# matwilso/generative_models

Hardware: AMD Instinct MI355X
Metric: ddpm_train_images_per_sec (higher is better)
Workload: dtype fp16_fwd+bf16_bwd; 1 GPU; DDPM train step, 3x32x32, SimpleUnet C=128, 2048 images per GPU, T=1000 (BASELINE.json configs[2]); key=cfg2, global_batch=2048, parallelism=dp1

## Files before the change

generative_models_amd/csrc/conv1x1_stream.hip:

```cpp
#include <type_traits>

#include "gmk_common.h"
#include "conv_plan.h"

namespace {

constexpr int kRow = 272;

template <typename T>
__global__ __launch_bounds__(256) void conv1x1_pair_stream_kernel(const T* __restrict__ src, const T* __restrict__ w, T* __restrict__ out_a,
                                                                 T* __restrict__ out_b, unsigned npix, unsigned ntiles, unsigned src_bytes) {
    fp16_saturating_stores<T>();
    typedef typename Frag16<T>::type frag_t;
    typedef __attribute__((ext_vector_type(4))) unsigned int u32x4s;
    constexpr unsigned kBadOff = 0xFFFFFF00u;
    __shared__ __attribute__((aligned(16))) char wl[256 * kRow];
    __shared__ __attribute__((aligned(16))) char tile[128 * kRow];
    __shared__ __attribute__((aligned(16))) char trans[4 * 32 * kRow];
    const int tid = threadIdx.x, lane = tid & 63, wave = tid >> 6;
    const int r = lane & 31, h = lane >> 5;
    const __amdgpu_buffer_rsrc_t rss = __builtin_amdgcn_make_buffer_rsrc(const_cast<T*>(src), 0, (int)src_bytes, 0x00020000);
    const __amdgpu_buffer_rsrc_t rsa = __builtin_amdgcn_make_buffer_rsrc(out_a, 0, (int)src_bytes, 0x00020000);
    const __amdgpu_buffer_rsrc_t rsb = __builtin_amdgcn_make_buffer_rsrc(out_b, 0, (int)src_bytes, 0x00020000);
#pragma unroll
// ... 126 lines not shown
    if (nk > 0) {
        load_step(0, ry[0], rx0[0], rx1[0]);
        if (nk > 1) load_step(1, ry[1], rx0[1], rx1[1]);
        write_step(0, ry[0], rx0[0], rx1[0]);
    }
    __syncthreads();
    auto k_step = [&](int ks, auto par) {
        constexpr int PAR = decltype(par)::value;
        if (ks + 2 < nk) load_step(ks + 2, ry[PAR], rx0[PAR], rx1[PAR]);
        const char* Yb = smem + PAR * 49152;
        const char* Xb = Yb + 16384 + cib * 16384;
#pragma unroll
        for (int kk = 0; kk < 4; ++kk) {
            bf16x8 a[2], b[2];
            const int pxl = kk * 16 + 8 * hh + q;
#pragma unroll
            for (int i = 0; i < 2; ++i) {
                const int wa = (((wm * 2 + i) ^ q) << 6) + 32 * cblk + 8 * pp;
                const int wb = (((wn * 2 + i) ^ q) << 6) + 32 * cblk + 8 * pp;
                s16x4 lo = __builtin_amdgcn_ds_read_tr16_b64_v4i16((GMK_LDS s16x4*)(Yb + pxl * 256 + wa));
                s16x4 hi = __builtin_amdgcn_ds_read_tr16_b64_v4i16((GMK_LDS s16x4*)(Yb + (pxl + 4) * 256 + wa));
                const s16x8 t = {lo[0], lo[1], lo[2], lo[3], hi[0], hi[1], hi[2], hi[3]};
                a[i] = __builtin_bit_cast(bf16x8, t);
                lo = __builtin_amdgcn_ds_read_tr16_b64_v4i16((GMK_LDS s16x4*)(Xb + pxl * 256 + wb));
                hi = __builtin_amdgcn_ds_read_tr16_b64_v4i16((GMK_LDS s16x4*)(Xb + (pxl + 4) * 256 + wb));
                const s16x8 u = {lo[0], lo[1], lo[2], lo[3], hi[0], hi[1], hi[2], hi[3]};
                b[i] = __builtin_bit_cast(bf16x8, u);
            }
#pragma unroll
            for (int i = 0; i < 2; ++i)
#pragma unroll
                for (int j = 0; j < 2; ++j) acc[i][j] = __builtin_amdgcn_mfma_f32_32x32x16_bf16(a[i], b[j], acc[i][j], 0, 0, 0);
        }
        if (ks + 1 < nk) write_step(PAR ^ 1, ry[PAR ^ 1], rx0[PAR ^ 1], rx1[PAR ^ 1]);
        __syncthreads();
    };
    for (int ks = 0; ks < nk; ks += 2) {
        k_step(ks, std::integral_constant<int, 0>{});
        if (ks + 1 < nk) k_step(ks + 1, std::integral_constant<int, 1>{});
    }
    float* out = slab + (int64_t)blockIdx.x * (128 * 256) + cib * 128;
#pragma unroll
    for (int i = 0; i < 2; ++i)
#pragma unroll
        for (int j = 0; j < 2; ++j)
#pragma unroll
            for (int e = 0; e < 16; ++e) {
                const int co = wm * 64 + i * 32 + (e & 3) + 8 * (e >> 2) + 4 * h;
                const int ci = wn * 64 + j * 32 + r;
                out[co * 256 + ci] = acc[i][j][e];
            }
}

}

int gmk_conv1x1_pair_stream_try(const void* src, int64_t npix, const void* w_rows256, void* out_a, void* out_b, int dtype, void* stream) {
    if (!gmk_is16(dtype) || gmk_kernel_choice(3, "GMK_DEV_VARIANT") == 46) return 0;
    const int64_t bytes = npix * 256;
    if (bytes >= 0xFFFFFF00ll) return 0;
    const int64_t ntiles = (npix + 127) / 128;
    const int ncu = gmk_cu_limit();
    if (ntiles < 2 * ncu) return 0;
    const unsigned grid = (unsigned)ncu;
    if (dtype == GMK_BF16)
        conv1x1_pair_stream_kernel<bf16_t><<<grid, 256, 0, gmk_stream(stream)>>>((const bf16_t*)src, (const bf16_t*)w_rows256, (bf16_t*)out_a, (bf16_t*)out_b,
                                                                    (unsigned)npix, (unsigned)ntiles, (unsigned)bytes);
    else
        conv1x1_pair_stream_kernel<f16_t><<<grid, 256, 0, gmk_stream(stream)>>>((const f16_t*)src, (const f16_t*)w_rows256, (f16_t*)out_a, (f16_t*)out_b,
                                                                   (unsigned)npix, (unsigned)ntiles, (unsigned)bytes);
    return 1;
}

int gmk_conv1x1_wgrad_stream_try(const void* dy, int dy_cstride, const void* src0, const void* src1, int64_t npix, float* slab, int64_t slab_bytes,
                                 bool x_f16, void* stream) {
    if (gmk_kernel_choice(3, "GMK_DEV_VARIANT") == 47) return 0;
    const int ncu = gmk_cu_limit();
    if (npix < (int64_t)ncu * 64 * 8 || npix >= (1ll << 31) - 64) return 0;
    if (slab_bytes < (int64_t)ncu * 128 * 256 * 4) return 0;
    int64_t chunk = (npix + ncu - 1) / ncu;
    chunk = (chunk + 63) / 64 * 64;
    const int ns = (int)((npix + chunk - 1) / chunk);
    if (x_f16)
        conv1x1_wgrad_stream_kernel<f16_t><<<ns, 512, 0, gmk_stream(stream)>>>((const bf16_t*)dy, dy_cstride, (const f16_t*)src0, (const f16_t*)src1, slab, (int)npix, (int)chunk);
    else
        conv1x1_wgrad_stream_kernel<bf16_t><<<ns, 512, 0, gmk_stream(stream)>>>((const bf16_t*)dy, dy_cstride, (const bf16_t*)src0, (const bf16_t*)src1, slab, (int)npix, (int)chunk);
    return ns;
}
```

generative_models_amd/csrc/conv_igemm.hip:

```cpp
#include <stdlib.h>

#include <type_traits>

#include "gmk_common.h"
#include "conv_plan.h"

namespace {

constexpr int kBM = 128, kBN = 128;

struct GatherParams {
    int hs, ws;
    int ho, wo;
    int ksize, pad;
    int mul, shift, mask, lim_h, lim_w;
    signed char ty[9], tx[9];
    unsigned char tapw[9];
    int ntaps;
    int oscale, ooy, oox, out_w, out_hw;
};

__host__ bool make_gather(int mode, int ksize, int hs, int ws, int ho, int wo, GatherParams* g) {
    g->hs = hs; g->ws = ws; g->ho = ho; g->wo = wo;
    g->ksize = ksize; g->pad = ksize == 3 ? 1 : 0;
// ... 1093 lines not shown
    call.c0 = c0; call.c1 = c1; call.B = B; call.hs = call.ho = H; call.ws = call.wo = W; call.ksize = 3; call.mode = GMK_CONV_NORMAL;
    call.w_rows = call.cout = call.out_cstride = cout; call.dtype = GMK_BF16; call.gn_scale = call.gn_shift = true; call.gn_stride = c0 + c1;
    return gmk_conv_route(call, gmk_kernel_choice(0, "GMK_CONV_KERNEL"), gmk_subpixel_enabled()).route == GMK_ROUTE_HALO;
}

extern "C" int gmk_conv_wgrad(const void* dy, int dy_cstride, const void* src0, const void* src1, int c0, int c1, int B,
                              int hs, int ws, int ho, int wo, int ksize, int mode, float* dw, int cout, void* workspace,
                              int64_t workspace_bytes, int dtype, int x_dtype, void* stream) {
    GMK_REQUIRE(dy && src0 && dw && workspace, "gmk_conv_wgrad: null pointer");
    GMK_REQUIRE(dtype == GMK_BF16 || dtype == GMK_F32, "gmk_conv_wgrad: bad dtype %d", dtype);
    GMK_REQUIRE(x_dtype == dtype || (dtype == GMK_BF16 && x_dtype == GMK_F16),
                "gmk_conv_wgrad: activations of type %d with gradients of type %d (same type, or fp16 activations with bf16 gradients)", x_dtype, dtype);
    const bool xf16 = x_dtype == GMK_F16;
    GMK_REQUIRE(ksize == 1 || ksize == 3, "gmk_conv_wgrad: ksize %d", ksize);
    GMK_REQUIRE(c0 > 0 && c0 % 128 == 0 && c1 >= 0 && c1 % 128 == 0 && (c1 == 0 || src1),
                "gmk_conv_wgrad: source channels must be multiples of 128 (c0=%d c1=%d)", c0, c1);
    GMK_REQUIRE(cout > 0 && cout % 128 == 0 && dy_cstride >= cout, "gmk_conv_wgrad: bad cout=%d", cout);
    GMK_REQUIRE(B > 0 && (int64_t)B * ho * wo < (1ll << 31) - 256 && (int64_t)B * hs * ws < (1ll << 31),
                "gmk_conv_wgrad: problem too large for 32-bit pixel indices");
    GMK_REQUIRE(mode != GMK_CONV_TRANSPOSED2, "gmk_conv_wgrad: no weight gradient for the transposed gather");
    WgradParams p = {};
    GMK_REQUIRE(make_gather(mode, ksize, hs, ws, ho, wo, &p.g), "gmk_conv_wgrad: mode %d inconsistent with %dx%d -> %dx%d", mode, hs, ws, ho, wo);
    const int taps = ksize * ksize;
    const int wforce = gmk_kernel_choice(1, "GMK_WGRAD_KERNEL");
    const bool s2 = mode == GMK_CONV_STRIDE2 && hs == 2 * ho && ws == 2 * wo;
    if (wforce != 1 && dtype == GMK_BF16 && (mode == GMK_CONV_NORMAL || mode == GMK_CONV_UPSAMPLE2 || s2) && ksize == 3) {
        const int ns2 = gmk_conv_wgrad_slots_try(dy, dy_cstride, src0, src1, c0, c1, B, ho, wo, cout, (float*)workspace,
                                                 workspace_bytes, wforce, mode == GMK_CONV_UPSAMPLE2, xf16, stream, s2);
        if (ns2 > 0) return wgrad_reduce("gmk_conv_wgrad(slots)", (const float*)workspace, dw, ns2, taps, cout, c0 + c1, stream);
    }
    if (wforce != 1 && ksize == 1 && mode == GMK_CONV_NORMAL && dtype == GMK_BF16 && c0 == 128 && c1 == 128 && cout == 128) {
        const int ns1 = gmk_conv1x1_wgrad_stream_try(dy, dy_cstride, src0, src1, (int64_t)B * ho * wo, (float*)workspace, workspace_bytes, xf16, stream);
        if (ns1 > 0) {
            gmk_note_kernel(GMK_K_CONV1X1_WGRAD_STREAM);
            return wgrad_reduce("gmk_conv_wgrad(1x1 stream)", (const float*)workspace, dw, ns1, 1, cout, 256, stream);
        }
    }
    p.dy = dy; p.dy_cstride = dy_cstride; p.src0 = src0; p.src1 = src1; p.c0 = c0; p.c1 = c1; p.ktot = c0 + c1;
    p.cout = cout; p.M = B * ho * wo;
    const int ns = wgrad_nsplit(p.M, taps, cout, p.ktot, &p.chunk);
    const int64_t need = (int64_t)ns * taps * cout * p.ktot * 4;
    GMK_REQUIRE(workspace_bytes >= need, "gmk_conv_wgrad: workspace %lld < %lld bytes", (long long)workspace_bytes,
                (long long)need);
    p.slab = (float*)workspace;
    gmk_note_kernel(GMK_K_CONV_WGRAD);
    p.ns = ns; p.taps = taps; p.order = (gmk_kernel_choice(3, "GMK_DEV_VARIANT") & 0xFF) == 61;
    dim3 grid((ns + 7) / 8 * 8 * taps * (cout / 128) * (p.ktot / 128));
    if (dtype == GMK_BF16 && xf16) conv_wgrad_kernel<bf16_t, f16_t><<<grid, 256, 0, gmk_stream(stream)>>>(p);
    else if (dtype == GMK_BF16) conv_wgrad_kernel<bf16_t><<<grid, 256, 0, gmk_stream(stream)>>>(p);
    else if (fp32_split()) conv_wgrad_kernel<float, float, true><<<grid, 256, 0, gmk_stream(stream)>>>(p);
    else conv_wgrad_kernel<float><<<grid, 256, 0, gmk_stream(stream)>>>(p);
    return wgrad_reduce("gmk_conv_wgrad", p.slab, dw, ns, taps, cout, p.ktot, stream);
}
```

generative_models_amd/csrc/conv_plan.h:

```cpp
#pragma once
#include <stdint.h>

#include "../../include/gmk.h"

static inline bool gmk_fits32(int64_t bytes) { return bytes < 0xFFFF0000ll; }
static inline bool gmk_halo_family_allowed(int conv_choice) { return conv_choice == 0 || conv_choice == 3; }
static inline int gmk_xcd_splits(int ns) {
    if (ns >= 8) {
        const int all8 = ns & ~7, two = ns & ~3;
        ns = all8 * 16 < ns * 15 ? two : all8;
    }
    return ns < 1 ? 1 : ns;
}

struct HaloGeometry { int R, TP, slots; int64_t rows_total, M, ntiles, nb0, nb1, nbw, nbo; };
int gmk_halo_geometry(int B, int H, int W, int c0, int c1, int w_rows, int cout, int out_cstride, int min_tiles, int upsample,
                      int fused_gn, HaloGeometry* g);

void gmk_halo_schedule(int64_t ntiles, int cu_limit, int variant, bool fold, int* grid_x, int* nfull, int* nhalf);
int gmk_conv3x3_halo_try(const void* src0, const void* src1, int c0, int c1, int B, int H, int W, const void* w, int w_rows,
                         int n0, int cout, const float* bias, const float* emb, int emb_stride, const void* residual,
                         void* out, int out_cstride, int min_tiles, int upsample, float* stats, int64_t stats_bytes,
                         const float* gn_scale, const float* gn_shift, int gn_stride, int dtype, void* stream);

bool gmk_subpixel_enabled(void);
int gmk_subpixel_plan(int B, int H, int W, int cin, int cout, int w_rows, int ntaps, int out_cstride, HaloGeometry* g);
int gmk_subpixel_takes(int conv_choice, bool subpixel_on, int B, int H, int W, int cin, int cout, int w_rows, int ntaps, int out_cstride, int dtype);

enum ConvRoute {
    GMK_ROUTE_SUBPIXEL,
    GMK_ROUTE_HALO,
    GMK_ROUTE_PHASES,
    GMK_ROUTE_NEEDS_HALO,
    GMK_ROUTE_DMA,
    GMK_ROUTE_REG,
    GMK_ROUTE_TWO_CALLS
};
struct ConvCall {
    int c0, c1, B, hs, ws, ho, wo, ksize, mode, w_rows, n0, cout, out_cstride, dtype;
    bool emb, out2, gn_stats, gn_scale, gn_shift;
    int gn_stride;
};
struct ConvRoutePlan {
    ConvRoute route;
    bool stuffed;
    int halo_min_tiles, halo_upsample;
    int64_t nb0, nb1, nbw, nbo;
};
ConvRoutePlan gmk_conv_route(const ConvCall& c, int conv_choice, bool subpixel_on);

struct SlotPlan {
    int kernel;
    bool wide, share;
    bool auto_ok;
    int WE, RE, nchunks;
    int ns_cu, ns, cps;
    int grid[3];
    int64_t nbdy, nb0, nb1, slab_bytes;
};
int gmk_wgrad_slots_nsplit(int cout, int ktot, int cu_limit);
int gmk_wgrad_slot_plan(int B, int H, int W, int c0, int c1, int cout, int dy_cstride, int forced, int upsample, bool x_f16, int stride2,
                        int cu_limit, SlotPlan* plan);
int gmk_conv_wgrad_slots_try(const void* dy, int dy_cstride, const void* src0, const void* src1, int c0, int c1, int B, int H,
                             int W, int cout, float* slab, int64_t slab_bytes, int forced, int upsample, bool x_f16,
                             void* stream, int stride2 = 0);

struct SubWgradPlan { int ns, cps, nchunks; int grid[3]; int64_t slab_bytes; };
int gmk_wgrad_subpixel_plan(int B, int H, int W, int cin, int cout, int dy_cstride, int cu_limit, SubWgradPlan* plan);

int gmk_conv1x1_pair_stream_try(const void* src, int64_t npix, const void* w_rows256, void* out_a, void* out_b, int dtype, void* stream);
int gmk_conv1x1_wgrad_stream_try(const void* dy, int dy_cstride, const void* src0, const void* src1, int64_t npix, float* slab, int64_t slab_bytes,
                                 bool x_f16, void* stream);

struct SmallPlan {
    int kernel, launches;
    unsigned grid, block, lds;
    int ppb, tps, band, nbands, rows;
    unsigned nblocks, ntiles, ppw;
};
int gmk_expand_plan(int B, int cs, int H, int W, int C, int dtype, int variant, int cu_limit, SmallPlan* p);
int gmk_wgrad3_plan(int B, int cs, int H, int W, int C, int dtype, int variant, int cu_limit, SmallPlan* p);
int gmk_head_plan(int B, int cs, int H, int W, int C, int dtype, int variant, int cu_limit, bool stem_dgrad, SmallPlan* p);
```

generative_models_amd/diffusion/simple_unet.py:

```python
import math
import os
from collections import OrderedDict

import torch
from torch import nn

from .. import ops

MAX_TIMESTEPS = 256


def _res_names(prefix, cin, cout, emb):
    out = [
        (f"{prefix}.in_layers.0.weight", (cin,)), (f"{prefix}.in_layers.0.bias", (cin,)),
        (f"{prefix}.in_layers.2.weight", (cout, cin, 3, 3)), (f"{prefix}.in_layers.2.bias", (cout,)),
        (f"{prefix}.emb_layers.1.weight", (cout, emb)), (f"{prefix}.emb_layers.1.bias", (cout,)),
        (f"{prefix}.out_layers.0.weight", (cout,)), (f"{prefix}.out_layers.0.bias", (cout,)),
        (f"{prefix}.out_layers.3.weight", (cout, cout, 3, 3)), (f"{prefix}.out_layers.3.bias", (cout,)),
    ]
    if cin != cout:
        out += [(f"{prefix}.skip_connection.weight", (cout, cin, 1, 1)), (f"{prefix}.skip_connection.bias", (cout,))]
    return out


# ... 527 lines not shown

    def _wgrad(self, dy, srcs, ksize, mode, dw):
        self._on_side(lambda: ops.conv_wgrad(dy, srcs, ksize, mode, dw), (dy, *srcs))
        return dw

    def _on_side(self, fn, tensors):
        if not ops.WGRAD_STREAM:
            return fn()
        if self._side is None:
            self._side = torch.cuda.Stream(device=tensors[0].device)
        side = self._side
        side.wait_stream(torch.cuda.current_stream())
        part = self._cu_part
        if part is not None:
            ops.set_cu_limit(part[1])
        try:
            with torch.cuda.stream(side):
                fn()
        finally:
            if part is not None:
                ops.set_cu_limit(part[0] - part[1])
        for t in tensors:
            t.record_stream(side)

    def _emb_ready(self):
        pend = getattr(self, "_emb_pending", None)
        if pend is not None:
            self._emb_pending = None
            self._join_side()
            pend.record_stream(torch.cuda.current_stream())

    def _join_side(self):
        if self._side is not None:
            torch.cuda.current_stream().wait_stream(self._side)

    def _res_bwd(self, name, ctx, dout, dout_sum, demb_all, blk, extra_add=None, grads=True, defer_skip=False):
        P, G, C = self._pv, self._gv, self.channels
        srcs, a, stats1, h, a2, (mean2, rstd2) = ctx.pop(name)
        B, H, W, _ = dout.shape
        two = len(srcs) == 2
        if grads:
            ops.colsum(dout_sum, G[f"{name}.out_layers.3.bias"], defer=True)
            self._wgrad(dout, [a2], 3, ops.NORMAL, G[f"{name}.out_layers.3.weight"])
        _, wd2 = self._packs[f"{name}.out_layers.3"]
        da2 = self._conv([dout], wd2, C, 3, ops.NORMAL, (H, W))
        dh, dgp, dbp = ops.gn_silu_bwd(da2, h, P[f"{name}.out_layers.0.weight"], P[f"{name}.out_layers.0.bias"], mean2,
                                       rstd2, dxsum=demb_all[:, blk * C:(blk + 1) * C] if grads else None,
                                       dropout=ctx.pop(name + ".dropout", None), xadd=ctx["emb_all"][:, blk * C:(blk + 1) * C])
        if grads:
            ops.colsum(dgp, G[f"{name}.out_layers.0.weight"], defer=True); ops.colsum(dbp, G[f"{name}.out_layers.0.bias"], defer=True)
            ops.colsum(demb_all[:, blk * C:(blk + 1) * C], G[f"{name}.in_layers.2.bias"], defer=True)
            self._wgrad(dh, a, 3, ops.NORMAL, G[f"{name}.in_layers.2.weight"])
        _, wd1 = self._packs[f"{name}.in_layers.2"]
        if two:
            if grads:
                ops.colsum(dout_sum, G[f"{name}.skip_connection.bias"], defer=True)
                self._wgrad(dout, srcs, 1, ops.NORMAL, G[f"{name}.skip_connection.weight"])
            _, wds = self._packs[f"{name}.skip_connection"]
        outs = []
        gw, gb = G[f"{name}.in_layers.0.weight"], G[f"{name}.in_layers.0.bias"]
        if two and C == 128:
            dskips = ops.conv1x1_pair(dout, wds, 2 * C)
        elif two:
            dskips = tuple(self._conv([dout], wds, 2 * C, 1, ops.NORMAL, (H, W), n0=i * C) for i in range(2))
        else:
            dskips = (dout,)
        for i, s in enumerate(srcs):
            da = self._conv([dh], wd1, len(srcs) * C, 3, ops.NORMAL, (H, W), n0=i * C)
            dskip = dskips[i]
            add2 = extra_add[i] if extra_add is not None else None
            gn = (da, dskip, P[f"{name}.in_layers.0.weight"][i * C:(i + 1) * C], P[f"{name}.in_layers.0.bias"][i * C:(i + 1) * C],
                  stats1[i][0], stats1[i][1])
            if defer_skip and i == 1 and grads and C == 128 and not self._narrow and ops.gn_pair_ok(s, self._g2, self._g1, da.dtype):
                outs.append((_DeferredGN(s, gn, gw[C:2 * C], gb[C:2 * C]), None))
                continue
            ssum = torch.empty((B, C), device=dout.device, dtype=torch.float32) if grads else None
            if isinstance(add2, _DeferredGN):
                assert add2.x is s
                ds, (ugp, ubp), (dgp, dbp) = ops.gn_silu_bwd_pair(s, add2.gn, gn, dxsum=ssum)
                ops.colsum(ugp, add2.gw, defer=True); ops.colsum(ubp, add2.gb, defer=True)
            else:
                ds, dgp, dbp = ops.gn_silu_bwd(da, s, *gn[2:], dadd1=dskip, dadd2=add2, dxsum=ssum)
            if grads:
                ops.colsum(dgp, gw[i * C:(i + 1) * C], defer=True); ops.colsum(dbp, gb[i * C:(i + 1) * C], defer=True)
            outs.append((ds, ssum))
        return outs

    def prepare_forward(self, dev=None):
        if self._packs_stale or self._packed_version != self._version_sum():
            self._repack()
        dev = self.flat_params.device if dev is None else dev
        self._freq_table(MAX_TIMESTEPS, dev)
        self._freq_table(4, dev)

    def forward_hip(self, x, logsnr, guide=None, cond_w=None, ctx=None, want_nu=False):
        if want_nu and not self.learn_var:
            raise ValueError("forward_hip: want_nu on a network without the variance head (learn_var)")
        if self._packs_stale or self._packed_version != self._version_sum():
            self._repack()
        P, C, T = self._pv, self.channels, self.act_dtype
        B, cin, H, W = x.shape
        if cin != self.in_channels or H % 4 or W % 4:
            raise ValueError(f"input {tuple(x.shape)}: need {self.in_channels} channels and H, W divisible by 4")
        x = ops.aligned(x.float())
        logsnr, guide, cond_w = ops.aligned(logsnr), ops.aligned(guide), ops.aligned(cond_w)
        if ops.EMB_SIDE and ops.WGRAD_STREAM and x.is_cuda and not torch.cuda.is_current_stream_capturing():
            box = []
            self._on_side(lambda: box.append(self._embed_fwd(logsnr, guide, cond_w, ctx)), tuple(t for t in (logsnr, guide, cond_w) if t is not None))
            emb_all = box[0]
            self._emb_pending = emb_all
        else:
            emb_all = self._embed_fwd(logsnr, guide, cond_w, ctx)
        H2, W2, H4, W4 = H // 2, W // 2, H // 4, W // 4
        t0 = ops.stem_fwd(x, P["down.seq.0.conv.weight"], P["down.seq.0.conv.bias"], C, T)
# ... 212 lines not shown
```

generative_models_amd/ops.py:

```python
import functools
import math

import os

import torch

from ._lib import C, K, check, kernel_name, lib

F32, BF16, F16 = C["GMK_F32"], C["GMK_BF16"], C["GMK_F16"]
_DT = {torch.float32: F32, torch.bfloat16: BF16, torch.float16: F16}
_HALF = (torch.bfloat16, torch.float16)
NORMAL, STRIDE2, UPSAMPLE2, TRANSPOSED2 = C["GMK_CONV_NORMAL"], C["GMK_CONV_STRIDE2"], C["GMK_CONV_UPSAMPLE2"], C["GMK_CONV_TRANSPOSED2"]

PROFILE = None


def instantiation_key(name, dtype):
    if dtype not in _HALF:
        return None
    t = "f16" if dtype == torch.float16 else "bf16"
    if name == "conv3x3_halo_ws_kernel":
        return f"{name}<{t}>"
    if name == "conv3x3_halo_ws_kernel[+1x1 skip]":
        return f"conv3x3_halo_ws_kernel<{t},+skip>"
# ... 443 lines not shown
    assert w.numel() == 9 * cout * c0 and wsk.numel() == cout * 2 * cs, (w.numel(), wsk.numel())
    _f32(bias, "bias"); _f32(bias_sk, "bias_sk")
    assert bias.numel() == cout and bias_sk.numel() == cout
    out = torch.empty((B, H, W, cout), device=s0.device, dtype=s0.dtype)
    with _Timed("conv_igemm", 2.0 * B * H * W * cout * (9 * c0 + 2 * cs), _nbytes(s0, k0, k1, out), dtype=s0.dtype):
        check(lib.gmk_conv3x3_skipfold(_p(s0), c0, B, H, W, _p(w), cout, 0, cout, _p(bias), _p(k0), _p(k1), cs, _p(wsk), cout, 0,
                                       _p(bias_sk), _p(out), cout, _DT[s0.dtype], _s()), "conv3x3_skipfold")
    return out


def conv1x1_pair(src, w, w_rows, n0=0):
    s0 = _chk(src, name="src")
    B, H, W, c = s0.shape
    _chk(w, s0.dtype, "w")
    assert w.numel() == w_rows * c and n0 + 256 <= w_rows
    oa = torch.empty((B, H, W, 128), device=s0.device, dtype=s0.dtype)
    ob = torch.empty_like(oa)
    with _Timed("conv_igemm", 2.0 * B * H * W * 256 * c, _nbytes(s0, oa, ob)):
        check(lib.gmk_conv1x1_pair(_p(s0), c, B, H, W, _p(w), w_rows, n0, _p(oa), _p(ob), _DT[s0.dtype], _s()), "conv1x1_pair")
    return oa, ob


_WS = {}


def _workspace(nbytes, device, tag="conv"):
    key = (tag, device.index, _s())
    ws = _WS.get(key)
    if ws is None or ws.numel() < nbytes:
        ws = torch.empty(int(nbytes), device=device, dtype=torch.uint8)
        _WS[key] = ws
    return ws


def conv_wgrad(dy, srcs, ksize, mode, dw):
    _chk(dy, name="dy")
    s0 = _chk(srcs[0], name="src0")
    s1 = _chk(srcs[1], s0.dtype, "src1") if len(srcs) > 1 else None
    assert s0.dtype == dy.dtype or (s0.dtype == torch.float16 and dy.dtype == torch.bfloat16), (s0.dtype, dy.dtype)
    B, hs, ws_, c0 = s0.shape
    c1 = s1.shape[3] if s1 is not None else 0
    _, ho, wo, cout = dy.shape
    assert dy.shape[0] == B
    assert dw.dtype == torch.float32 and dw.is_contiguous() and dw.numel() == cout * (c0 + c1) * ksize * ksize
    need = lib.gmk_conv_wgrad_workspace_bytes(B * ho * wo, ksize * ksize, cout, c0 + c1)
    assert need > 0
    wsbuf = _workspace(need, dy.device)
    with _Timed("conv_wgrad", 2.0 * B * ho * wo * cout * (c0 + c1) * ksize * ksize, _nbytes(dy, s0, s1)):
        check(lib.gmk_conv_wgrad(_p(dy), cout, _p(s0), _p(s1), c0, c1, B, hs, ws_, ho, wo, ksize, mode, _p(dw), cout,
                                 _p(wsbuf), wsbuf.numel(), _DT[dy.dtype], _DT[s0.dtype], _s()), "conv_wgrad")
    return dw


def conv_wgrad_subpixel_ok(B, H, W, c, dy_dtype, cout=128):
    return dy_dtype == torch.bfloat16 and bool(lib.gmk_conv_wgrad_subpixel_ok(B, H, W, c, cout))


def conv_wgrad_subpixel(dy, x, dw):
    _chk(dy, torch.bfloat16, "dy")
    _chk(x, name="x")
    assert x.dtype in _HALF
    B, H, W, cin = x.shape
    cout = dy.shape[3]
    assert dy.shape == (B, 2 * H, 2 * W, cout)
    assert dw.dtype == torch.float32 and dw.is_contiguous() and dw.numel() == cout * cin * 9
    need = lib.gmk_conv_wgrad_subpixel_workspace_bytes(B, H, W, cin, cout)
    assert need > 0
    wsbuf = _workspace(need, dy.device)
    with _Timed("conv_wgrad", 2.0 * B * 4 * H * W * cout * cin * 9, _nbytes(dy, x), multiplied=2.0 * B * H * W * cout * cin * 16):
        check(lib.gmk_conv_wgrad_subpixel(_p(dy), cout, _p(x), B, H, W, cin, cout, _p(dw), _p(wsbuf), wsbuf.numel(), _DT[dy.dtype],
                                          _DT[x.dtype], _s()), "conv_wgrad_subpixel")
    return dw


def stem_fwd(x, w, bias, C, dtype):
    _f32(x, "x"); _f32(w, "w"); _f32(bias, "bias")
    B, cin, H, W = x.shape
    assert w.shape == (C, cin, 3, 3)
    y = torch.empty((B, H, W, C), device=x.device, dtype=dtype)
    with _Timed("stem_fwd", 2.0 * B * H * W * C * cin * 9, _nbytes(x, y)):
        check(lib.gmk_stem_fwd(_p(x), _p(w), _p(bias), _p(y), B, cin, H, W, C, _DT[dtype], _s()), "stem_fwd")
    return y


def stem_wgrad(x, dy, dw):
    _f32(x, "x"); _chk(dy, name="dy")
    B, cin, H, W = x.shape
    C = dy.shape[3]
    nb = lib.gmk_stem_wgrad_blocks(B * H * W)
    part = torch.empty((nb, C * cin * 9), device=x.device, dtype=torch.float32)
    with _Timed("stem_wgrad", 2.0 * B * H * W * C * cin * 9, _nbytes(x, dy)):
        check(lib.gmk_stem_wgrad(_p(x), _p(dy), _p(part), B, cin, H, W, C, _DT[dy.dtype], _s()), "stem_wgrad")
    return colsum(part, dw)


def head_fwd(a, w, bias):
    _chk(a, name="a"); _f32(w, "w"); _f32(bias, "bias")
    B, H, W, C = a.shape
    cout = w.shape[0]
    assert w.shape == (cout, C, 3, 3)
    out = torch.empty((B, cout, H, W), device=a.device, dtype=torch.float32)
    with _Timed("head_fwd", 2.0 * B * H * W * C * cout * 9, _nbytes(a, out)):
        check(lib.gmk_head_fwd(_p(a), _p(w), _p(bias), _p(out), B, cout, H, W, C, _DT[a.dtype], _s()), "head_fwd")
    return out


# ... 999 lines not shown
```

include/gmk.h:

```cpp
#ifndef GMK_H
#define GMK_H
#include <stdint.h>

#ifdef __cplusplus
extern "C" {
#endif

#define GMK_F32 0
#define GMK_BF16 1
#define GMK_F16 2
#define GMK_ERR_ARG (-1)

#define GMK_CONV_NORMAL 0
#define GMK_CONV_STRIDE2 1
#define GMK_CONV_UPSAMPLE2 2
#define GMK_CONV_TRANSPOSED2 3

int gmk_version(void);
const char* gmk_last_error(void);
#define GMK_KERNEL_TABLE(X)                                                                                                               \
    X(CONV_IGEMM, 1, "conv_igemm_kernel")                                                                                                 \
    X(CONV_IGEMM_DMA, 2, "conv_igemm_dma_kernel")                                                                                         \
    X(CONV_HALO, 3, "conv3x3_halo_kernel")                                                                                                \
    X(CONV_HALO_WS, 4, "conv3x3_halo_ws_kernel")                                                                                          \
// ... 56 lines not shown
                    float drop_p, uint64_t drop_seed, uint64_t drop_offset, const float* xadd, int xadd_stride, int dtype,
                    void* stream);
int gmk_gn_silu_bwd(const void* dy, const void* x, const float* gamma, const float* beta, const float* mean,
                    const float* rstd, const void* dadd1, const void* dadd2, void* dx, float* dgamma_part,
                    float* dbeta_part, float* dxsum, int dxsum_stride, int B, int HW, int C, int groups,
                    float drop_p, uint64_t drop_seed, uint64_t drop_offset, const float* xadd, int xadd_stride, int dtype,
                    int x_dtype, void* stream);
int gmk_gn_pair_ok(int HW, int C, int groups_a, int groups_b, int x_dtype, int grad_dtype);
int gmk_gn_pair_fwd_ok(int HW, int C, int groups_a, int groups_b, int dtype);
int gmk_gn_silu_fwd_pair(const void* x, void* y_a, void* y_b, const float* gamma_a, const float* beta_a, const float* gamma_b,
                         const float* beta_b, float* mean_a, float* rstd_a, float* mean_b, float* rstd_b, int B, int HW, int C,
                         int groups_a, int groups_b, float eps, const float* xadd, int xadd_stride, int dtype, void* stream);
int gmk_gn_silu_bwd_pair(const void* x, const void* dy_up, const void* dadd_up, const float* gamma_up, const float* beta_up,
                         const float* mean_up, const float* rstd_up, float* dgamma_part_up, float* dbeta_part_up, int groups_up,
                         const void* dy_dn, const void* dadd_dn, const float* gamma_dn, const float* beta_dn, const float* mean_dn,
                         const float* rstd_dn, float* dgamma_part_dn, float* dbeta_part_dn, int groups_dn, void* dx, float* dxsum,
                         int dxsum_stride, int B, int HW, int C, const float* xadd, int xadd_stride, int x_dtype, void* stream);
int gmk_cast16(const void* src, void* dst, int64_t n, int src_dtype, int dst_dtype, void* stream);
int gmk_chansum(const void* x, float* out, int out_stride, int B, int HW, int C, int dtype, void* stream);
int gmk_colsum(const float* part, int64_t stride, float* out, int R, int C, int accumulate, void* stream);
int gmk_colsum_multi(int n, const float* const* part, const int64_t* stride, float* const* out, const int* R,
                     const int* C, void* stream);
int gmk_sumpool2x2(const void* x, void* y, int B, int H, int W, int C, int dtype, void* stream);

int gmk_conv_igemm(const void* src0, const void* src1, int c0, int c1, int B, int hs, int ws, int ho, int wo,
                   int ksize, int mode, const void* w, int w_rows, int n0, int cout, const float* bias,
                   const float* emb, int emb_stride, const void* residual, void* out, int out_cstride,
                   float* gn_stats, int64_t gn_stats_bytes, const float* gn_scale, const float* gn_shift, int gn_stride,
                   int dtype, void* stream);
int gmk_conv_gn_fusable(int B, int H, int W, int c0, int c1, int cout);
int gmk_conv1x1_pair(const void* src, int c, int B, int H, int W, const void* w, int w_rows, int n0, void* out_a, void* out_b,
                     int dtype, void* stream);
int gmk_conv3x3_skipfold_ok(int B, int H, int W, int c0, int cs, int cout);
int gmk_conv3x3_skipfold(const void* src, int c0, int B, int H, int W, const void* w, int w_rows, int n0, int cout,
                         const float* bias, const void* sk0, const void* sk1, int cs, const void* wsk, int wsk_rows, int nsk0,
                         const float* bias_sk, void* out, int out_cstride, int dtype, void* stream);
#define GMK_SUBPIXEL_UPSAMPLE 0
#define GMK_SUBPIXEL_TRANSPOSED 1
#define GMK_SUBPIXEL_UPSAMPLE_DGRAD 2
int gmk_conv_subpixel_ok(int B, int H, int W, int cin, int cout, int dtype);
int gmk_pack_upsample_weight(const float* w, void* w_sub, void* w_sub_dgrad, int cout, int cin, int dtype, int dgrad_dtype, void* stream);
int gmk_conv_subpixel(const void* src, int B, int H, int W, int cin, const void* w, int w_rows, int n0, int cout, int mode,
                      const float* bias, const void* residual, void* out, int out_cstride, int dtype, void* stream);
int gmk_conv_wgrad_subpixel_ok(int B, int H, int W, int cin, int cout);
int64_t gmk_conv_wgrad_subpixel_workspace_bytes(int B, int H, int W, int cin, int cout);
int gmk_conv_wgrad_subpixel(const void* dy, int dy_cstride, const void* x, int B, int H, int W, int cin, int cout, float* dw,
                            void* workspace, int64_t workspace_bytes, int dtype, int x_dtype, void* stream);
int gmk_gn_stats(const void* x, const float* gamma, const float* beta, float* mean, float* rstd, float* tab_scale,
                 float* tab_shift, int tab_stride, int B, int HW, int C, int groups, float eps, const float* xadd,
                 int xadd_stride, int dtype, void* stream);
int gmk_conv_wgrad(const void* dy, int dy_cstride, const void* src0, const void* src1, int c0, int c1, int B,
                   int hs, int ws, int ho, int wo, int ksize, int mode, float* dw, int cout, void* workspace,
                   int64_t workspace_bytes, int dtype, int x_dtype, void* stream);

int gmk_stem_fwd(const float* x, const float* w, const float* bias, void* y, int B, int cin, int H, int W, int C,
                 int dtype, void* stream);
int gmk_stem_wgrad_blocks(int64_t n_pixels);
int gmk_stem_wgrad(const float* x, const void* dy, float* dw_part, int B, int cin, int H, int W, int C, int dtype,
                   void* stream);
int gmk_head_fwd(const void* a, const float* w, const float* bias, float* out, int B, int cout, int H, int W, int C,
                 int dtype, void* stream);
int gmk_head_dgrad(const float* dout, const float* w, void* da, int B, int cout, int H, int W, int C, int dtype,
                   void* stream);
int gmk_head_wgrad_blocks(int64_t n_pixels);
int gmk_head_wgrad(const float* dout, const void* a, float* dw_part, int B, int cout, int H, int W, int C, int dtype,
                   void* stream);
int gmk_stem_dgrad(const void* dy, const float* w, float* dx, int B, int cin, int H, int W, int C, int dtype, void* stream);

int gmk_timestep_embedding(const float* t, const float* freqs, float* out, int B, void* stream);
int gmk_guide_onehot(const int64_t* guide, float* onehot, float* keep, int B, void* stream);
int gmk_label_drop(int64_t* y, int B, float p, uint64_t seed, uint64_t offset, void* stream);
int gmk_batch_gather(const uint8_t* images, const uint8_t* labels, const int64_t* index, int B, int64_t N, int C, int H, int W, int pad,
                     int binarize, float flip_p, uint64_t seed, uint64_t offset, float* x, int64_t* y, void* stream);
int gmk_to_uint8(const float* x, uint8_t* out, int64_t n_images, int C, int H, int W, int crop, void* stream);
int gmk_image_grid(const float* x, uint8_t* out, int T, int N, int C, int H, int W, int crop, int ncol, int gap, int fill, int out_channels,
                   int row_prefix, void* stream);
int gmk_mean(const float* x, int n, float* out, void* stream);
int gmk_gemm_f32(const float* A, int64_t sa0, int64_t sa1, const float* B, int64_t sb0, int64_t sb1, float* C,
                 int64_t ldc, int M, int N, int K, const float* bias, const float* bias2, const float* rowscale,
                 int silu, int accumulate, void* workspace, int64_t workspace_bytes, void* stream);
int64_t gmk_gemm_f32_workspace_bytes(int M, int N, int K);
int gmk_silu_bwd(const float* dpost, const float* pre, const float* rowscale, float* dpre, int64_t n, int ncols,
                 void* stream);
int gmk_scale_rows(const float* in, const float* rowscale, float* out, int64_t n, int ncols, void* stream);

int gmk_rng_normal(float* out, int64_t n, uint64_t seed, uint64_t offset, void* stream);
int gmk_rng_uniform(float* out, int64_t n, uint64_t seed, uint64_t offset, void* stream);
int gmk_q_sample(const float* x, const float* eps, const float* u, float* logsnr, float* z, int B, int64_t n,
                 void* stream);
#define GMK_SCHED_COSINE 0
#define GMK_SCHED_UNIFORM 1
#define GMK_SCHED_BETA_CONST 2
#define GMK_SCHED_BETA_LINEAR 3
int gmk_q_sample_sched(const float* x, const float* eps, const float* u, float* logsnr, float* z, int B, int64_t n, int kind, float a,
                       float b, float lmin, float lmax, float shift, void* stream);
#define GMK_MEAN_V 0
#define GMK_MEAN_EPS 1
#define GMK_MEAN_X 2
int gmk_v_loss(const float* v, const float* z, const float* x, const float* eps, const float* logsnr, float* loss_b,
               float* x_mse, float* eps_mse, float* dv, float grad_scale, int loss_type, int mean_type, int B, int64_t n,
               void* stream);
#define GMK_LOSS_W_SNR_PLUS1 0
#define GMK_LOSS_W_MIN_SNR 1
#define GMK_X_LOSS_KEEP 12288
int gmk_x_loss_w(const float* v, const float* z, const float* x, const float* logsnr, float* loss_b, float* x_mse, float* dv,
                 float grad_scale, int weight_type, float gamma, int mean_type, int B, int64_t n, void* stream);
// ... 119 lines not shown
```

Before: 46940 images/s.

## Fuse skip-connection 1x1 conv dgrad and wgrad into one streaming backward kernel

Adds a streaming kernel that reads dout and both source tensors once per pixel tile. From that single pass it computes the skip-connection weight gradient (accumulated into per-block slabs) and the two dgrad outputs, which are staged through LDS. This replaces separate conv1x1_pair and wgrad launches that each re-read dout, cutting memory traffic and a launch. The price is higher LDS and register pressure in one larger kernel. The eligibility checks are also moved into shared inline plan helpers.

```diff
diff --git a/generative_models_amd/csrc/conv1x1_stream.hip b/generative_models_amd/csrc/conv1x1_stream.hip
--- a/generative_models_amd/csrc/conv1x1_stream.hip
+++ b/generative_models_amd/csrc/conv1x1_stream.hip
@@ -202,15 +202,174 @@
             }
 }
 
+template <typename TX>
+__global__ __launch_bounds__(512) void conv1x1_bwd_stream_kernel(const bf16_t* __restrict__ dy, int dy_cstride, const TX* __restrict__ src0,
+                                                                const TX* __restrict__ src1, const bf16_t* __restrict__ w, bf16_t* __restrict__ out_a,
+                                                                bf16_t* __restrict__ out_b, float* __restrict__ slab, int M, int chunk) {
+    typedef __attribute__((ext_vector_type(4))) unsigned int u32x4s;
+    typedef __attribute__((ext_vector_type(8))) short s16x8;
+    constexpr int kStep = 3 * 16384, kStage = 64 * 512;
+    __shared__ __attribute__((aligned(16))) char smem[2 * kStep + 2 * kStage];
+    char* const stage = smem + 2 * kStep;
+    const int tid = threadIdx.x, lane = tid & 63, wave = tid >> 6;
+    const int wm = wave >> 2, wq = wave & 3, cib = wq >> 1, wn = wq & 1;
+    const int pix_begin = blockIdx.x * chunk;
+    const int pix_end = min(pix_begin + chunk, M);
+    const int nk = pix_end > pix_begin ? (pix_end - pix_begin + 63) / 64 : 0;
+    const int r = lane & 31, h = lane >> 5;
+    bf16x8 wf[8];
+#pragma unroll
+    for (int kk = 0; kk < 8; ++kk) wf[kk] = *reinterpret_cast<const bf16x8*>(w + (wave * 32 + r) * 128 + 16 * kk + 8 * h);
+    int lds_w[2], srow[2];
+    const int sc = tid & 15;
+#pragma unroll
+    for (int j = 0; j < 2; ++j) {
+        const int row = (tid >> 4) + 32 * j;
+        srow[j] = row;
+        lds_w[j] = row * 256 + ((((sc >> 2) ^ (row & 3)) << 2 | (sc & 3)) << 4);
+    }
+    u32x4s ry[2][2], rx0[2][2], rx1[2][2];
+    auto load_step = [&](int ks, u32x4s (&y)[2], u32x4s (&x0)[2], u32x4s (&x1)[2]) {
+#pragma unroll
+        for (int j = 0; j < 2; ++j) {
+            const int m = pix_begin + ks * 64 + srow[j];
+            u32x4s vy = {0u, 0u, 0u, 0u}, v0 = vy, v1 = vy;
+            if (m < pix_end) {
+                vy = *reinterpret_cast<const u32x4s*>(dy + (int64_t)m * dy_cstride + sc * 8);
+                v0 = *reinterpret_cast<const u32x4s*>(src0 + (int64_t)m * 128 + sc * 8);
+                v1 = *reinterpret_cast<const u32x4s*>(src1 + (int64_t)m * 128 + sc * 8);
+            }
+            y[j] = vy; x0[j] = v0; x1[j] = v1;
+        }
+    };
+    auto round_x = [&](u32x4s v) {
+        if constexpr (!__is_same(TX, bf16_t)) {
+#pragma unroll
+            for (int d = 0; d < 4; ++d) {
+                float lo, hi;
+                unpack_pair<TX>(v[d], lo, hi);
+                v[d] = pack_pair<bf16_t>(lo, hi);
+            }
+        }
+        return v;
+    };
+    auto write_step = [&](int buf, const u32x4s (&y)[2], const u32x4s (&x0)[2], const u32x4s (&x1)[2]) {
+        char* b = smem + buf * kStep;
+#pragma unroll
+        for (int j = 0; j < 2; ++j) {
+            *reinterpret_cast<u32x4s*>(b + lds_w[j]) = y[j];
+            *reinterpret_cast<u32x4s*>(b + 16384 + lds_w[j]) = round_x(x0[j]);
+            *reinterpret_cast<u32x4s*>(b + 32768 + lds_w[j]) = round_x(x1[j]);
+        }
+    };
+    auto store_step = [&](int ks, int buf) {
+        const char* s = stage + buf * kStage;
+#pragma unroll
+        for (int half = 0; half < 2; ++half)
+#pragma unroll
+            for (int j = 0; j < 2; ++j) {
+                const int row = srow[j], m = pix_begin + ks * 64 + row;
+                const u32x4s v = *reinterpret_cast<const u32x4s*>(s + row * 512 + (((half * 16 + sc) ^ (row & 7)) << 4));
+                if (m < pix_end) *reinterpret_cast<u32x4s*>((half ? out_b : out_a) + (int64_t)m * 128 + sc * 8) = v;
+            }
+    };
+    f32x16 acc[2][2];
+#pragma unroll
+    for (int i = 0; i < 2; ++i)
+#pragma unroll
+        for (int j = 0; j < 2; ++j)
+#pragma unroll
+            for (int e = 0; e < 16; ++e) acc[i][j][e] = 0.f;
+    const int gg = lane >> 4, i16 = lane & 15, q = i16 >> 2, pp = i16 & 3;
+    const int hh = gg >> 1, cblk = gg & 1;
+    if (nk > 0) {
+        load_step(0, ry[0], rx0[0], rx1[0]);
+        if (nk > 1) load_step(1, ry[1], rx0[1], rx1[1]);
+        write_step(0, ry[0], rx0[0], rx1[0]);
+    }
+    __syncthreads();
+    auto k_step = [&](int ks, auto par) {
+        constexpr int PAR = decltype(par)::value;
+        if (ks + 2 < nk) load_step(ks + 2, ry[PAR], rx0[PAR], rx1[PAR]);
+        if (ks > 0) store_step(ks - 1, PAR ^ 1);
+        const char* Yb = smem + PAR * kStep;
+        const char* Xb = Yb + 16384 + cib * 16384;
+#pragma unroll
+        for (int kk = 0; kk < 4; ++kk) {
+            bf16x8 a[2], b[2];
+            const int pxl = kk * 16 + 8 * hh + q;
+#pragma unroll
+            for (int i = 0; i < 2; ++i) {
+                const int wa = (((wm * 2 + i) ^ q) << 6) + 32 * cblk + 8 * pp;
+                const int wb = (((wn * 2 + i) ^ q) << 6) + 32 * cblk + 8 * pp;
+                s16x4 lo = __builtin_amdgcn_ds_read_tr16_b64_v4i16((GMK_LDS s16x4*)(Yb + pxl * 256 + wa));
+                s16x4 hi = __builtin_amdgcn_ds_read_tr16_b64_v4i16((GMK_LDS s16x4*)(Yb + (pxl + 4) * 256 + wa));
+                const s16x8 t = {lo[0], lo[1], lo[2], lo[3], hi[0], hi[1], hi[2], hi[3]};
+                a[i] = __builtin_bit_cast(bf16x8, t);
+                lo = __builtin_amdgcn_ds_read_tr16_b64_v4i16((GMK_LDS s16x4*)(Xb + pxl * 256 + wb));
+                hi = __builtin_amdgcn_ds_read_tr16_b64_v4i16((GMK_LDS s16x4*)(Xb + (pxl + 4) * 256 + wb));
+                const s16x8 u = {lo[0], lo[1], lo[2], lo[3], hi[0], hi[1], hi[2], hi[3]};
+                b[i] = __builtin_bit_cast(bf16x8, u);
+            }
+#pragma unroll
+            for (int i = 0; i < 2; ++i)
+#pragma unroll
+                for (int j = 0; j < 2; ++j) acc[i][j] = __builtin_amdgcn_mfma_f32_32x32x16_bf16(a[i], b[j], acc[i][j], 0, 0, 0);
+        }
+        char* sg = stage + PAR * kStage;
+#pragma unroll
+        for (int pb = 0; pb < 2; ++pb) {
+            const int row = pb * 32 + r;
+            f32x16 d;
+#pragma unroll
+            for (int e = 0; e < 16; ++e) d[e] = 0.f;
+#pragma unroll
+            for (int kk = 0; kk < 8; ++kk) {
+                const int c = 2 * kk + h;
+                const bf16x8 bfr = *reinterpret_cast<const bf16x8*>(Yb + row * 256 + ((((c >> 2) ^ (row & 3)) << 2 | (c & 3)) << 4));
+                d = mfma_32x32x16<bf16_t>(wf[kk], bfr, d);
+            }
+            unsigned pk[4][2];
+#pragma unroll
+            for (int q4 = 0; q4 < 4; ++q4) {
+                pk[q4][0] = pack_pair<bf16_t>(sat16<bf16_t>(d[4 * q4]), sat16<bf16_t>(d[4 * q4 + 1]));
+                pk[q4][1] = pack_pair<bf16_t>(sat16<bf16_t>(d[4 * q4 + 2]), sat16<bf16_t>(d[4 * q4 + 3]));
+            }
+#pragma unroll
+            for (int q4 = 0; q4 < 4; q4 += 2) {
+                const auto s0 = __builtin_amdgcn_permlane32_swap(pk[q4][0], pk[q4 + 1][0], false, false);
+                const auto s1 = __builtin_amdgcn_permlane32_swap(pk[q4][1], pk[q4 + 1][1], false, false);
+                const u32x4s o = {s0[0], s1[0], s0[1], s1[1]};
+                *reinterpret_cast<u32x4s*>(sg + row * 512 + (((wave * 4 + q4 + h) ^ (row & 7)) << 4)) = o;
+            }
+        }
+        if (ks + 1 < nk) write_step(PAR ^ 1, ry[PAR ^ 1], rx0[PAR ^ 1], rx1[PAR ^ 1]);
+        __syncthreads();
+    };
+    for (int ks = 0; ks < nk; ks += 2) {
+        k_step(ks, std::integral_constant<int, 0>{});
+        if (ks + 1 < nk) k_step(ks + 1, std::integral_constant<int, 1>{});
+    }
+    if (nk > 0) store_step(nk - 1, (nk - 1) & 1);
+    float* out = slab + (int64_t)blockIdx.x * (128 * 256) + cib * 128;
+#pragma unroll
+    for (int i = 0; i < 2; ++i)
+#pragma unroll
+        for (int j = 0; j < 2; ++j)
+#pragma unroll
+            for (int e = 0; e < 16; ++e) {
+                const int co = wm * 64 + i * 32 + (e & 3) + 8 * (e >> 2) + 4 * h;
+                const int ci = wn * 64 + j * 32 + r;
+                out[co * 256 + ci] = acc[i][j][e];
+            }
+}
+
 }
 
 int gmk_conv1x1_pair_stream_try(const void* src, int64_t npix, const void* w_rows256, void* out_a, void* out_b, int dtype, void* stream) {
-    if (!gmk_is16(dtype) || gmk_kernel_choice(3, "GMK_DEV_VARIANT") == 46) return 0;
-    const int64_t bytes = npix * 256;
-    if (bytes >= 0xFFFFFF00ll) return 0;
-    const int64_t ntiles = (npix + 127) / 128;
     const int ncu = gmk_cu_limit();
-    if (ntiles < 2 * ncu) return 0;
+    if (!gmk_conv1x1_pair_stream_ok(npix, dtype, gmk_kernel_choice(3, "GMK_DEV_VARIANT"), ncu)) return 0;
+    const int64_t bytes = npix * 256, ntiles = (npix + 127) / 128;
     const unsigned grid = (unsigned)ncu;
     if (dtype == GMK_BF16)
         conv1x1_pair_stream_kernel<bf16_t><<<grid, 256, 0, gmk_stream(stream)>>>((const bf16_t*)src, (const bf16_t*)w_rows256, (bf16_t*)out_a, (bf16_t*)out_b,
@@ -223,16 +382,25 @@
 
 int gmk_conv1x1_wgrad_stream_try(const void* dy, int dy_cstride, const void* src0, const void* src1, int64_t npix, float* slab, int64_t slab_bytes,
                                  bool x_f16, void* stream) {
-    if (gmk_kernel_choice(3, "GMK_DEV_VARIANT") == 47) return 0;
-    const int ncu = gmk_cu_limit();
-    if (npix < (int64_t)ncu * 64 * 8 || npix >= (1ll << 31) - 64) return 0;
-    if (slab_bytes < (int64_t)ncu * 128 * 256 * 4) return 0;
-    int64_t chunk = (npix + ncu - 1) / ncu;
-    chunk = (chunk + 63) / 64 * 64;
-    const int ns = (int)((npix + chunk - 1) / chunk);
+    StreamWgradPlan p;
+    if (!gmk_conv1x1_wgrad_stream_plan(npix, gmk_kernel_choice(3, "GMK_DEV_VARIANT"), gmk_cu_limit(), &p) || slab_bytes < p.slab_bytes) return 0;
+    const int ns = p.ns, chunk = p.chunk;
     if (x_f16)
         conv1x1_wgrad_stream_kernel<f16_t><<<ns, 512, 0, gmk_stream(stream)>>>((const bf16_t*)dy, dy_cstride, (const f16_t*)src0, (const f16_t*)src1, slab, (int)npix, (int)chunk);
     else
         conv1x1_wgrad_stream_kernel<bf16_t><<<ns, 512, 0, gmk_stream(stream)>>>((const bf16_t*)dy, dy_cstride, (const bf16_t*)src0, (const bf16_t*)src1, slab, (int)npix, (int)chunk);
     return ns;
 }
+
+int gmk_conv1x1_bwd_stream_try(const void* dy, int dy_cstride, const void* src0, const void* src1, const void* w_rows256, void* dskip_a, void* dskip_b,
+                               int64_t npix, float* slab, int64_t slab_bytes, bool x_f16, void* stream) {
+    StreamWgradPlan p;
+    if (!gmk_conv1x1_bwd_stream_plan(npix, gmk_kernel_choice(3, "GMK_DEV_VARIANT"), gmk_cu_limit(), slab_bytes, &p)) return 0;
+    if (x_f16)
+        conv1x1_bwd_stream_kernel<f16_t><<<p.ns, 512, 0, gmk_stream(stream)>>>((const bf16_t*)dy, dy_cstride, (const f16_t*)src0, (const f16_t*)src1, (const bf16_t*)w_rows256,
+                                                                              (bf16_t*)dskip_a, (bf16_t*)dskip_b, slab, (int)npix, p.chunk);
+    else
+        conv1x1_bwd_stream_kernel<bf16_t><<<p.ns, 512, 0, gmk_stream(stream)>>>((const bf16_t*)dy, dy_cstride, (const bf16_t*)src0, (const bf16_t*)src1, (const bf16_t*)w_rows256,
+                                                                               (bf16_t*)dskip_a, (bf16_t*)dskip_b, slab, (int)npix, p.chunk);
+    return p.ns;
+}
diff --git a/generative_models_amd/csrc/conv_igemm.hip b/generative_models_amd/csrc/conv_igemm.hip
--- a/generative_models_amd/csrc/conv_igemm.hip
+++ b/generative_models_amd/csrc/conv_igemm.hip
@@ -1169,3 +1169,24 @@
     else conv_wgrad_kernel<float><<<grid, 256, 0, gmk_stream(stream)>>>(p);
     return wgrad_reduce("gmk_conv_wgrad", p.slab, dw, ns, taps, cout, p.ktot, stream);
 }
+
+extern "C" int gmk_conv1x1_bwd_ok(int B, int H, int W, int64_t workspace_bytes) {
+    StreamWgradPlan p;
+    return B > 0 && H > 0 && W > 0 &&
+           gmk_conv1x1_bwd_stream_plan((int64_t)B * H * W, gmk_kernel_choice(3, "GMK_DEV_VARIANT"), gmk_cu_limit(), workspace_bytes, &p);
+}
+
+extern "C" int gmk_conv1x1_bwd(const void* dy, int dy_cstride, const void* src0, const void* src1, int B, int H, int W, const void* w, int w_rows,
+                               int n0, void* dskip_a, void* dskip_b, float* dw, void* workspace, int64_t workspace_bytes, int x_dtype,
+                               void* stream) {
+    GMK_REQUIRE(dy && src0 && src1 && w && dskip_a && dskip_b && dw && workspace, "gmk_conv1x1_bwd: null pointer");
+    GMK_REQUIRE(x_dtype == GMK_BF16 || x_dtype == GMK_F16, "gmk_conv1x1_bwd: sources of type %d (bf16 or fp16 beside bf16 gradients)", x_dtype);
+    GMK_REQUIRE(dy_cstride >= 128 && dy_cstride % 8 == 0, "gmk_conv1x1_bwd: bad dy_cstride=%d", dy_cstride);
+    GMK_REQUIRE(n0 >= 0 && n0 + 256 <= w_rows, "gmk_conv1x1_bwd: rows n0 .. n0 + 255 outside the %d packed rows", w_rows);
+    GMK_REQUIRE(B > 0 && H > 0 && W > 0, "gmk_conv1x1_bwd: bad shape");
+    const int ns = gmk_conv1x1_bwd_stream_try(dy, dy_cstride, src0, src1, (const char*)w + (size_t)n0 * 128 * 2, dskip_a, dskip_b, (int64_t)B * H * W,
+                                              (float*)workspace, workspace_bytes, x_dtype == GMK_F16, stream);
+    GMK_REQUIRE(ns > 0, "gmk_conv1x1_bwd: B=%d %dx%d is not taken (see gmk_conv1x1_bwd_ok): call gmk_conv1x1_pair and gmk_conv_wgrad", B, H, W);
+    gmk_note_kernel(0);
+    return wgrad_reduce("gmk_conv1x1_bwd", (const float*)workspace, dw, ns, 1, 128, 256, stream);
+}
diff --git a/generative_models_amd/csrc/conv_plan.h b/generative_models_amd/csrc/conv_plan.h
--- a/generative_models_amd/csrc/conv_plan.h
+++ b/generative_models_amd/csrc/conv_plan.h
@@ -71,6 +71,28 @@
 int gmk_conv1x1_pair_stream_try(const void* src, int64_t npix, const void* w_rows256, void* out_a, void* out_b, int dtype, void* stream);
 int gmk_conv1x1_wgrad_stream_try(const void* dy, int dy_cstride, const void* src0, const void* src1, int64_t npix, float* slab, int64_t slab_bytes,
                                  bool x_f16, void* stream);
+static inline bool gmk_conv1x1_pair_stream_ok(int64_t npix, int dtype, int variant, int cu_limit) {
+    if ((dtype != GMK_BF16 && dtype != GMK_F16) || variant == 46) return false;
+    if (npix * 256 >= 0xFFFFFF00ll) return false;
+    return (npix + 127) / 128 >= 2 * (int64_t)cu_limit;
+}
+struct StreamWgradPlan { int ns, chunk; int64_t slab_bytes; };
+static inline bool gmk_conv1x1_wgrad_stream_plan(int64_t npix, int variant, int cu_limit, StreamWgradPlan* p) {
+    if (variant == 47) return false;
+    if (npix < (int64_t)cu_limit * 64 * 8 || npix >= (1ll << 31) - 64) return false;
+    int64_t chunk = (npix + cu_limit - 1) / cu_limit;
+    chunk = (chunk + 63) / 64 * 64;
+    p->chunk = (int)chunk;
+    p->ns = (int)((npix + chunk - 1) / chunk);
+    p->slab_bytes = (int64_t)cu_limit * 128 * 256 * 4;
+    return true;
+}
+static inline bool gmk_conv1x1_bwd_stream_plan(int64_t npix, int variant, int cu_limit, int64_t slab_bytes, StreamWgradPlan* p) {
+    return variant != 48 && gmk_conv1x1_pair_stream_ok(npix, GMK_BF16, variant, cu_limit) && gmk_conv1x1_wgrad_stream_plan(npix, variant, cu_limit, p) &&
+           slab_bytes >= p->slab_bytes;
+}
+int gmk_conv1x1_bwd_stream_try(const void* dy, int dy_cstride, const void* src0, const void* src1, const void* w_rows256, void* dskip_a, void* dskip_b,
+                               int64_t npix, float* slab, int64_t slab_bytes, bool x_f16, void* stream);
 
 struct SmallPlan {
     int kernel, launches;
diff --git a/generative_models_amd/diffusion/simple_unet.py b/generative_models_amd/diffusion/simple_unet.py
--- a/generative_models_amd/diffusion/simple_unet.py
+++ b/generative_models_amd/diffusion/simple_unet.py
@@ -603,14 +603,20 @@
             ops.colsum(demb_all[:, blk * C:(blk + 1) * C], G[f"{name}.in_layers.2.bias"], defer=True)
             self._wgrad(dh, a, 3, ops.NORMAL, G[f"{name}.in_layers.2.weight"])
         _, wd1 = self._packs[f"{name}.in_layers.2"]
+        dskips = None
         if two:
+            _, wds = self._packs[f"{name}.skip_connection"]
             if grads:
                 ops.colsum(dout_sum, G[f"{name}.skip_connection.bias"], defer=True)
-                self._wgrad(dout, srcs, 1, ops.NORMAL, G[f"{name}.skip_connection.weight"])
-            _, wds = self._packs[f"{name}.skip_connection"]
+                if C == 128 and ops.conv1x1_bwd_ok(dout, srcs):
+                    dskips = ops.conv1x1_bwd(dout, srcs, wds, G[f"{name}.skip_connection.weight"])
+                else:
+                    self._wgrad(dout, srcs, 1, ops.NORMAL, G[f"{name}.skip_connection.weight"])
         outs = []
         gw, gb = G[f"{name}.in_layers.0.weight"], G[f"{name}.in_layers.0.bias"]
-        if two and C == 128:
+        if dskips is not None:
+            pass
+        elif two and C == 128:
             dskips = ops.conv1x1_pair(dout, wds, 2 * C)
         elif two:
             dskips = tuple(self._conv([dout], wds, 2 * C, 1, ops.NORMAL, (H, W), n0=i * C) for i in range(2))
diff --git a/generative_models_amd/ops.py b/generative_models_amd/ops.py
--- a/generative_models_amd/ops.py
+++ b/generative_models_amd/ops.py
@@ -519,6 +519,45 @@
     return dw
 
 
+def _skip_bwd_view(dout):
+    B, H, W, c = dout.shape
+    cs = dout.stride(2)
+    if not dout.is_cuda or dout.dtype != torch.bfloat16 or c != 128 or dout.data_ptr() % 16:
+        raise ValueError(f"conv1x1_bwd: dout {tuple(dout.shape)} of {dout.dtype}: a 16-byte aligned bf16 device tensor of 128 channels")
+    if dout.stride(3) != 1 or cs < 128 or cs % 8 or dout.stride(1) != W * cs or dout.stride(0) != H * W * cs:
+        raise ValueError(f"conv1x1_bwd: dout strides {dout.stride()}: NHWC with a channel stride of 128 or more")
+    return cs
+
+
+def conv1x1_bwd_ok(dout, srcs):
+    if len(srcs) != 2 or dout.dtype != torch.bfloat16 or dout.shape[3] != 128 or any(s.shape[3] != 128 or s.dtype not in _HALF for s in srcs):
+        return False
+    B, H, W, _ = dout.shape
+    return bool(lib.gmk_conv1x1_bwd_ok(B, H, W, lib.gmk_conv_wgrad_workspace_bytes(B * H * W, 1, 128, 256)))
+
+
+def conv1x1_bwd(dout, srcs, wds, dw):
+    cs = _skip_bwd_view(dout)
+    s0 = _chk(srcs[0], name="src0")
+    s1 = _chk(srcs[1], s0.dtype, "src1")
+    _chk(wds, torch.bfloat16, "wds")
+    B, H, W, _ = dout.shape
+    assert s0.dtype in _HALF and s0.shape == s1.shape == (B, H, W, 128) and wds.numel() == 256 * 128
+    assert dw.dtype == torch.float32 and dw.is_contiguous() and dw.numel() == 128 * 256
+    if not conv1x1_bwd_ok(dout, srcs):
+        dskips = conv1x1_pair(dout, wds, 256)
+        conv_wgrad(dout, srcs, 1, NORMAL, dw)
+        return dskips
+    wsbuf = _workspace(lib.gmk_conv_wgrad_workspace_bytes(B * H * W, 1, 128, 256), dout.device)
+    oa = torch.empty((B, H, W, 128), device=dout.device, dtype=dout.dtype)
+    ob = torch.empty_like(oa)
+    npix = B * H * W
+    with _Timed("conv1x1_bwd_stream_kernel", 2 * 2.0 * npix * 128 * 256, 5 * npix * 256, fixed=True):
+        check(lib.gmk_conv1x1_bwd(_p(dout), cs, _p(s0), _p(s1), B, H, W, _p(wds), 256, 0, _p(oa), _p(ob), _p(dw), _p(wsbuf), wsbuf.numel(),
+                                  _DT[s0.dtype], _s()), "conv1x1_bwd")
+    return oa, ob
+
+
 def conv_wgrad_subpixel_ok(B, H, W, c, dy_dtype, cout=128):
     return dy_dtype == torch.bfloat16 and bool(lib.gmk_conv_wgrad_subpixel_ok(B, H, W, c, cout))
 
diff --git a/include/gmk.h b/include/gmk.h
--- a/include/gmk.h
+++ b/include/gmk.h
@@ -132,6 +132,9 @@
 int gmk_conv_wgrad(const void* dy, int dy_cstride, const void* src0, const void* src1, int c0, int c1, int B,
                    int hs, int ws, int ho, int wo, int ksize, int mode, float* dw, int cout, void* workspace,
                    int64_t workspace_bytes, int dtype, int x_dtype, void* stream);
+int gmk_conv1x1_bwd_ok(int B, int H, int W, int64_t workspace_bytes);
+int gmk_conv1x1_bwd(const void* dy, int dy_cstride, const void* src0, const void* src1, int B, int H, int W, const void* w, int w_rows,
+                    int n0, void* dskip_a, void* dskip_b, float* dw, void* workspace, int64_t workspace_bytes, int x_dtype, void* stream);
 
 int gmk_stem_fwd(const float* x, const float* w, const float* bias, void* y, int B, int cin, int H, int W, int C,
                  int dtype, void* stream);
```

Measured after the change: 47200 images/s, median of 6. Within noise of the previous version (+0.6%).
